# cvxopt/smcp

Hardware: AMD Instinct MI355X
Metric: Newton KKT solves/sec (higher is better)
Workload: dtype f64; 1 GPU; synth50k nested block-arrow SDP n=50000, 8073 cliques, m=100; kktsolver=chol, n=50000, cliques=8073, m=100, blkval_doubles=2493568, update_doubles=10689536, parallelism=single

## Files before the change

smcp_amd/csrc/capi.hip:

```cpp
#include <hip/hip_runtime.h>
#include <memory>
#include <unordered_map>

#include <algorithm>
#include <chrono>
#include <cstdio>
#include <cstring>
#include <map>
#include <new>
#include <atomic>
#include <thread>
#include <type_traits>
#include <vector>

#include "../../include/smcp_amd.h"
#include "context.hpp"
#include "switches.hpp"
#include "front_generic.hip"
#include "front_mfma.hip"
#include "front_large.hip"
#include "front_top.hip"
#include "front_inv.hip"
#include "front_n16.hip"
#include "front_downfam.hip"
// ... 336 lines not shown
  }
}

inline unsigned gather_parts(int namax, int64_t pairs = (int64_t)1 << 40, int ncu = 0) {
  const int base = std::max(1, std::min(64, (namax * namax) / (NT * 32)));
  if (pairs * base >= 2 * (int64_t)ncu) return (unsigned)base;
  const int cap = std::max(1, std::min(64, (namax * namax) / (NT * 2)));
  return (unsigned)std::max<int64_t>(base, std::min<int64_t>(cap, (2 * (int64_t)ncu + pairs - 1) / std::max<int64_t>(1, pairs)));
}
inline int namax_of(csp_ctx* c, const int32_t* lev) {
  const int64_t off = lev - c->D.levidx;
  const auto& lp = c->S.levptr;
  const int64_t l = std::upper_bound(lp.begin(), lp.end(), off) - lp.begin() - 1;
  return (l >= 0 && l < (int64_t)c->lev_namax.size()) ? c->lev_namax[l] : 0;
}

void gather_all(csp_ctx* c, const double* x, int64_t ldx, int nrhs, double* updbase, hipStream_t st) {
  TreeArgs a = tree_args(c);
  for_levels_down(c, [&](const int32_t* lev, int cnt) {
    a.lev = lev;
    launch(c, KID_gather_level, k_gather_level, dim3(cnt, nrhs, gather_parts(namax_of(c, lev), (int64_t)cnt * nrhs, c->D.ncu)), dim3(NT), st, a, x, ldx, updbase);
  });
}

int prepare_yaa(csp_ctx* c, const double* Y, bool need_fac, hipStream_t st, bool need_inv = false, bool allow_partial = false);
void complete_fac(csp_ctx* c, hipStream_t st);


constexpr size_t LDS_LIMIT = 160 * 1024 - 2048;

bool cache_off() {
  static int nocache = -1;
  if (nocache < 0) { const char* e = sw_str("SMCP_NOCACHE"); nocache = (e && e[0] == '1') ? 1 : 0; }
  return nocache == 1;
}

bool use_generic(const csp_ctx* c) {
  static int g = -1;
  if (g < 0) { const char* e = sw_str("SMCP_GENERIC"); g = (e && e[0] == '1') ? 1 : 0; }
  return g == 1 || (c && c->deterministic);
}

MfmaArgs mfma_args(csp_ctx* c, const double* ysc, int ymode, int nrhs) {
  MfmaArgs a;
  a.t = tree_args(c);
  a.t.lev = c->D.lev2idx;
  a.LK = c->D.lk;
  a.ysc = ysc;
  a.ymode = ymode;
  a.nnmax = a.namax = 0;
  a.nchmax = a.panmax = a.pkmax = a.plansum = 0;
  a.nrhs = nrhs;
  { static int sk = -1; if (sk < 0) { const char* e = sw_str("SMCP_SKIP"); sk = e ? atoi(e) : 0; } a.skip = sk; }
  a.dbg = (a.skip & 64) ? (unsigned long long*)(c->D.red + 768) : nullptr;
  a.lfd = c->D.lfd;
  a.dn = 0; a.dld = 0;
  a.kc_ptr = nullptr; a.kc_off = nullptr; a.kc_val = nullptr; a.kc_ids = nullptr;
  a.sp_rt = c->D.sp_rt; a.sp_mk = c->D.sp_mk;
  a.kc_stride = 0; a.kc_j0 = 0;
  a.nnmin = 0;
  a.grp_ptr = nullptr; a.grp_list = nullptr; a.chskip = nullptr; a.famt_ngrp = 0;
  a.fz_on = 0; a.fz_nat = 0; a.fz_cnn = 0; a.fz_stride = 0; a.fz_recl = 0;
  a.fz_tab = nullptr; a.fz_no = nullptr; a.fz_slot = nullptr; a.fz_ptr = nullptr; a.fz_pk = nullptr; a.fz_s = nullptr;
  a.level = 0; a.nS = 0; a.famna = a.fampan = a.fampk = a.famcna = a.famnn = a.famcnn = 0;
  return a;
}

int rhs_groups(int ncl, int nrhs, int target) {
  int g = (target + ncl - 1) / ncl;
  return std::max(1, std::min(g, nrhs));
}

template <class F>
void for_level_classes(csp_ctx* c, int64_t l, MfmaArgs a, F f, int set = 0) {
  const LevelClass& L = set ? c->sets[set].lvl[l] : c->lvl[l];
  const int32_t* base = set ? c->sets[set].lev2 + c->sets[set].off[l] : c->D.lev2idx + c->S.levptr[l];
  if (L.nI) {
    a.t.lev = base;
    a.nnmax = L.nnmaxI;
    a.namax = L.namaxI;
    a.nchmax = L.nchmaxI;
    a.panmax = L.panmaxI;
    a.pkmax = L.pkmaxI;
    a.plansum = L.plansumI;
    a.level = (int)l; a.nS = (int)L.nS; a.famna = L.famna; a.fampan = L.fampan; a.fampk = L.fampk; a.famcna = L.famcna; a.famnn = L.famnn; a.famcnn = L.famcnn;
    size_t lds = (size_t)mfma_lds_doubles(L.nnmaxI, L.namaxI) * sizeof(double);
    f(true, a, (int)L.nI, lds, lds > 48 * 1024 ? 512 : 256);
  }
  if (L.nII) {
    a.t.lev = base + L.nI;
    a.level = (int)l;
    a.nnmax = L.nnmaxII;
    a.nnmin = L.nnminII;
    a.namax = L.namaxII;
    a.nchmax = L.nchmaxII;
    f(false, a, (int)L.nII, (size_t)0, 1024);
  }
}


template <class F>
void for_all_large(csp_ctx* c, MfmaArgs a, F f) {
  if (!c->D.nII_total) return;
  a.t.lev = c->D.lev3idx + c->D.nI_total;
  a.nnmax = c->D.nnmaxII_all;
  a.namax = c->D.namaxII_all;
// ... 3332 lines not shown
```

smcp_amd/csrc/front_large.hip:

```cpp
#include <hip/hip_runtime.h>
#include <type_traits>

namespace smcp {

constexpr int LT = 64;
constexpr int LKC = 16;
constexpr int LSA = LT + 1, LSB = LKC + 1;

template <int PD>
__device__ inline double ldm(bool c, const double* p) {
  if constexpr (PD == 4) { const double v = *p; return c ? v : 0.0; }
  else return c ? *p : 0.0;
}
template <int PD = 1, class LA, class LB>
__device__ inline void gemm_tile64(d4 (&acc)[2][2], int M, int N, int Kd, int m0, int n0, LA la, LB lb,
                                   double* sA, double* sB, int kbeg = 0) {
  const int tid = threadIdx.x, lane = tid & 63, wave = tid >> 6;
  const int l15 = lane & 15, kq = lane >> 4;
  const int kfirst = (kbeg / LKC) * LKC;
  if (kfirst >= Kd) return;
  if constexpr (PD == 4) {
    const int wm = wave & 3, wn = wave >> 2;
    const int ia = tid & 63, ka = tid >> 6, kb = tid & 15, jb = tid >> 4;
    const int mi = max(0, min(m0 + ia, M - 1)), nj = max(0, min(n0 + jb, N - 1));
// ... 41 lines not shown
      vb[u] = (n0 + j < N && k0 + kb < Kd) ? lb(k0 + kb, n0 + j) : 0.0;
    }
  };
  fetch(kfirst);
  for (int k0 = kfirst; k0 < Kd; k0 += LKC) {
    __syncthreads();
#pragma unroll
    for (int u = 0; u < 4; ++u) {
      const int e = tid + 256 * u;
      sA[(e & 63) + (e >> 6) * LSA] = va[u];
      sB[(e & 15) + (e >> 4) * LSB] = vb[u];
    }
    __syncthreads();
    if (k0 + LKC < Kd) fetch(k0 + LKC);
#pragma unroll
    for (int ks = 0; ks < LKC / 4; ++ks) {
      const int kk = 4 * ks + kq;
      const double a0 = sA[(32 * wm + l15) + kk * LSA], a1 = sA[(32 * wm + 16 + l15) + kk * LSA];
      const double b0 = sB[kk + (32 * wn + l15) * LSB], b1 = sB[kk + (32 * wn + 16 + l15) * LSB];
      acc[0][0] = __builtin_amdgcn_mfma_f64_16x16x4f64(b0, a0, acc[0][0], 0, 0, 0);
      acc[1][0] = __builtin_amdgcn_mfma_f64_16x16x4f64(b0, a1, acc[1][0], 0, 0, 0);
      acc[0][1] = __builtin_amdgcn_mfma_f64_16x16x4f64(b1, a0, acc[0][1], 0, 0, 0);
      acc[1][1] = __builtin_amdgcn_mfma_f64_16x16x4f64(b1, a1, acc[1][1], 0, 0, 0);
    }
  }
  }
}
constexpr int LRC = 80;
constexpr int LCC = 18;
constexpr int LRC_DOUBLES = 4 * LKC * LRC;
__device__ inline bool rc_aligned(const double* p, int64_t ld) { return ((reinterpret_cast<uintptr_t>(p) & 15) == 0) && ((ld & 1) == 0); }
template <bool XC>
struct RcOperand {
  typedef double d2 __attribute__((ext_vector_type(2)));
  const double* p; int64_t step, second;
  int st0, st1;
  d2 r[2];
  __device__ inline void init(const double* X, int64_t ld) {
    const int tid = threadIdx.x;
    if constexpr (XC) {
      const int k2 = tid & 7, row = tid >> 3;
      p = X + 2 * k2 + (int64_t)row * ld; step = LKC; second = 32 * ld;
      st0 = 2 * k2 + row * LCC; st1 = st0 + 32 * LCC;
    } else {
      const int r2 = tid & 31, kk0 = tid >> 5;
      p = X + 2 * r2 + (int64_t)kk0 * ld; step = (int64_t)LKC * ld; second = 8 * ld;
      st0 = 2 * r2 + kk0 * LRC; st1 = st0 + 8 * LRC;
    }
  }
  __device__ inline void fetch() { r[0] = *reinterpret_cast<const d2*>(p); r[1] = *reinterpret_cast<const d2*>(p + second); p += step; }
  __device__ inline void stage(double* sX) const { *reinterpret_cast<d2*>(sX + st0) = r[0]; *reinterpret_cast<d2*>(sX + st1) = r[1]; }
  static __device__ inline double frag(const double* sX, int row, int kk) { return XC ? sX[kk + row * LCC] : sX[row + kk * LRC]; }
};
template <bool AC, bool BC>
__device__ inline void gemm_tile64_rc(d4 (&acc)[2][2], const double* A, int64_t lda, const double* B, int64_t ldb, int nk, double* smem) {
  constexpr int SL = LKC * LRC;
  const int tid = threadIdx.x, lane = tid & 63, wave = tid >> 6;
  const int l15 = lane & 15, kq = lane >> 4;
  const int wm = wave & 1, wn = wave >> 1;
  const int ns = nk / LKC;
  if (ns <= 0) return;
  RcOperand<AC> oa;
  RcOperand<BC> ob;
  oa.init(A, lda);
  ob.init(B, ldb);
  oa.fetch(); ob.fetch();
  __syncthreads();
  oa.stage(smem); ob.stage(smem + 2 * SL);
  __syncthreads();
  for (int s = 0; s < ns; ++s) {
    const double* sA = smem + (s & 1) * SL;
    const double* sB = smem + 2 * SL + (s & 1) * SL;
    if (s + 1 < ns) { oa.fetch(); ob.fetch(); }
#pragma unroll
    for (int ks = 0; ks < LKC / 4; ++ks) {
      const int kk = 4 * ks + kq;
      const double a0 = RcOperand<AC>::frag(sA, 32 * wm + l15, kk), a1 = RcOperand<AC>::frag(sA, 32 * wm + 16 + l15, kk);
      const double b0 = RcOperand<BC>::frag(sB, 32 * wn + l15, kk), b1 = RcOperand<BC>::frag(sB, 32 * wn + 16 + l15, kk);
      acc[0][0] = __builtin_amdgcn_mfma_f64_16x16x4f64(b0, a0, acc[0][0], 0, 0, 0);
      acc[1][0] = __builtin_amdgcn_mfma_f64_16x16x4f64(b0, a1, acc[1][0], 0, 0, 0);
      acc[0][1] = __builtin_amdgcn_mfma_f64_16x16x4f64(b1, a0, acc[0][1], 0, 0, 0);
      acc[1][1] = __builtin_amdgcn_mfma_f64_16x16x4f64(b1, a1, acc[1][1], 0, 0, 0);
    }
    if (s + 1 < ns) { oa.stage(smem + ((s + 1) & 1) * SL); ob.stage(smem + 2 * SL + ((s + 1) & 1) * SL); }
    __syncthreads();
  }
}
template <int PD, bool AC = false, bool BC = false>
__device__ inline void gemm_tile64_plain(d4 (&acc)[2][2], const double* A, int64_t lda, int M, const double* B, int64_t ldb, int N, int k0, int k1,
                                         int m0, int n0, double* smem) {
  if (k1 <= k0) return;
  if constexpr (PD == 1) {
    const double* A0 = AC ? A + k0 + (int64_t)m0 * lda : A + m0 + (int64_t)k0 * lda;
    const double* B0 = BC ? B + k0 + (int64_t)n0 * ldb : B + n0 + (int64_t)k0 * ldb;
    if (m0 + LT <= M && n0 + LT <= N && ((k1 - k0) % LKC) == 0 && (k0 % LKC) == 0 && rc_aligned(A0, lda) && rc_aligned(B0, ldb)) {
      gemm_tile64_rc<AC, BC>(acc, A0, lda, B0, ldb, k1 - k0, smem);
      return;
    }
  }
  gemm_tile64<PD>(acc, M, N, k1, m0, n0, [=](int m, int kk) { return AC ? A[kk + (int64_t)m * lda] : A[m + (int64_t)kk * lda]; },
                  [=](int kk, int n) { return BC ? B[kk + (int64_t)n * ldb] : B[n + (int64_t)kk * ldb]; }, smem, smem + LKC * LSA, k0);
}
__device__ inline bool tile64_pos(int a, int b, int r, int& m, int& n) {
  const int lane = threadIdx.x & 63, wave = threadIdx.x >> 6;
  const int l15 = lane & 15, kq = lane >> 4;
  if (blockDim.x == 1024) {
    m = 16 * (wave & 3) + l15; n = 16 * (wave >> 2) + kq + 4 * r;
    return a == 0 && b == 0;
  }
  m = 32 * (wave & 1) + 16 * a + l15; n = 32 * (wave >> 1) + 16 * b + kq + 4 * r;
  return true;
}
template <class F>
__device__ inline void tile64_foreach(const d4 (&acc)[2][2], int m0, int n0, int M, int N, F f) {
#pragma unroll
  for (int a = 0; a < 2; ++a)
#pragma unroll
    for (int b = 0; b < 2; ++b)
#pragma unroll
      for (int r = 0; r < 4; ++r) {
        int m, n;
        const bool has = tile64_pos(a, b, r, m, n);
        m += m0; n += n0;
        if (has && m < M && n < N) f(m, n, acc[a][b][r]);
      }
}
template <class LD, class ST>
__device__ inline void tile64_rmw(const d4 (&acc)[2][2], int m0, int n0, int M, int N, LD ld, ST st) {
  double old[2][2][4];
#pragma unroll
  for (int a = 0; a < 2; ++a)
#pragma unroll
    for (int b = 0; b < 2; ++b)
#pragma unroll
      for (int r = 0; r < 4; ++r) {
        int m, n;
        tile64_pos(a, b, r, m, n);
        old[a][b][r] = ld(max(0, min(m0 + m, M - 1)), max(0, min(n0 + n, N - 1)));
      }
#pragma unroll
  for (int a = 0; a < 2; ++a)
#pragma unroll
    for (int b = 0; b < 2; ++b)
#pragma unroll
      for (int r = 0; r < 4; ++r) {
        int m, n;
        const bool has = tile64_pos(a, b, r, m, n);
        m += m0; n += n0;
        if (has && m < M && n < N) st(m, n, acc[a][b][r], old[a][b][r]);
      }
}
__device__ inline void tile64_zero(d4 (&acc)[2][2]) {
#pragma unroll
  for (int a = 0; a < 2; ++a)
// ... 346 lines not shown
      const int cj = rel[j] - c0;
      const double* col = Uc + pk_col(j, nac) - j;
      for (int i = max(i0, j) + lane; i < i1; i += 64) unsafeAtomicAdd(&T[(rel[i] - r0) + cj * LF_TR], col[i]);
    }
  }
  __syncthreads();
  double* P = u + (int64_t)r * ldu + d.blk;
  double* U = a.t.upd + (int64_t)r * a.t.updlen + d.upd;
  const int nr = r1 - r0;
  for (int e = threadIdx.x; e < nr * (c1 - c0); e += blockDim.x) {
    const int i = r0 + e % nr, j = c0 + e / nr;
    if (i < j) continue;
    const double v = T[(i - r0) + (j - c0) * LF_TR];
    if (j < nn) {
      if (v != 0.0) P[i + (int64_t)j * nf] += (sgn == 1) ? -v : v;
    } else if (sgn) {
      if (v != 0.0) U[(i - nn) + (int64_t)(j - nn) * na] += v;
    } else {
      U[(i - nn) + (int64_t)(j - nn) * na] = v;
    }
  }
}
__global__ void k_lf_zero_skipped(MfmaArgs a) {
  const CliqueDesc d = a.t.cl[a.t.lev[blockIdx.x]];
  const int r = blockIdx.y;
  for (int q = d.chbeg; q < d.chend; ++q) {
    const int ck = a.t.chidx[q];
    if (!a.chskip[ck]) continue;
    const CliqueDesc c = a.t.cl[ck];
    double* UP = a.t.updp + (int64_t)r * a.t.updplen + c.updp;
    for (int e = threadIdx.x; e < c.na * (c.na + 1) / 2; e += blockDim.x) UP[e] = 0.0;
  }
}
__global__ void k_lf_clear_upd(MfmaArgs a) {
  const int k = a.t.lev[blockIdx.y];
  const CliqueDesc d = a.t.cl[k];
  double* U = a.t.upd + (int64_t)blockIdx.z * a.t.updlen + d.upd;
  const int64_t len = (int64_t)d.na * d.na;
  for (int64_t e = (int64_t)blockIdx.x * blockDim.x + threadIdx.x; e < len; e += (int64_t)gridDim.x * blockDim.x) U[e] = 0.0;
}

__host__ __device__ inline bool lf_sym_split(int nn) { return nn > 6 * LT; }
template <int PD>
__global__ void __launch_bounds__(PD == 4 ? 1024 : 256, 4) k_lf_up1(MfmaArgs a, double* u, int64_t ldu) {
  __shared__ __attribute__((aligned(16))) double smem[PD == 1 ? LRC_DOUBLES : LKC * LSA + LT * LSB];
  double* const sA = smem; double* const sB = smem + LKC * LSA;
  const LfCtx c = lf_ctx(a, u, ldu);
  const int nn = c.nn, na = c.na, nf = c.nf;
  const int mtA = tiles64(na), ntN = tiles64(nn);
  const int nE = mtA * ntN, nT = ntN * ntN;
  const int t = blockIdx.x;
  if (t >= nE + nT) return;
  const double* P = c.P;
  auto fsym = [=](int kk, int n) { return P[max(kk, n) + (int64_t)min(kk, n) * nf]; };
  d4 acc[2][2];
  tile64_zero(acc);
  if (t < nE) {
    const int m0 = (t % mtA) * LT, n0 = (t / mtA) * LT;
    const double* K = c.K;
    gemm_tile64<PD>(acc, na, nn, nn, m0, n0, [=](int m, int kk) { return K[m + (int64_t)kk * nf]; }, fsym, sA, sB);
    double* E = c.E; double* Pw = c.P;
    tile64_rmw(acc, m0, n0, na, nn, [=](int m, int n) { return Pw[nn + m + (int64_t)n * nf]; },
               [=](int m, int n, double v, double f) {
                 E[m + (int64_t)n * na] = f - 0.5 * v;
                 Pw[nn + m + (int64_t)n * nf] = f - v;
               });
  } else {
    const int tt = t - nE, m0 = (tt % ntN) * LT, n0 = (tt / ntN) * LT;
    const double* Li = c.Li;
    if (n0 > m0) return;
    if (lf_sym_split(nn)) {
      gemm_tile64<PD>(acc, nn, nn, min(nn, n0 + LT), m0, n0, [=](int m, int kk) { return Li[m + (int64_t)kk * nf]; },
                  [=](int kk, int n) { const double v_ = ldm<PD>(kk >= n, &P[kk + (int64_t)n * nf]); return kk == n ? 0.5 * v_ : v_; },
                  sA, sB, n0);
      gemm_tile64_plain<PD, false, true>(acc, Li, nf, nn, P, nf, nn, n0 + LT, min(nn, m0 + LT), m0, n0, smem);
    } else {
      gemm_tile64<PD>(acc, nn, nn, min(nn, m0 + LT), m0, n0, [=](int m, int kk) { return Li[m + (int64_t)kk * nf]; }, fsym, sA, sB);
    }
    double* T = c.T;
    tile64_foreach(acc, m0, n0, nn, nn, [=](int m, int n, double v) { T[m + (int64_t)n * nn] = v; });
  }
}
constexpr int LF_ZSP_MAXNN = 7168;
__global__ void __launch_bounds__(256) k_lf_zsp(MfmaArgs a, double* u, int64_t ldu) {
  extern __shared__ __attribute__((aligned(16))) double zc[];
  __shared__ int s_row[64];
  __shared__ double s_w[64];
  const LfCtx c = lf_ctx(a, u, ldu);
  const int nn = c.nn, nf = c.nf;
  const int col = blockIdx.x;
  if (col >= nn) return;
  const int tid = threadIdx.x;
  const int r0 = (col / LT) * LT;
  const int r = blockIdx.z;
  const int j = a.kc_ids ? a.kc_ids[a.kc_j0 + r] : a.kc_j0 + r;
  const int32_t* kp = a.kc_ptr + (int64_t)c.k * a.kc_stride;
  const int e0 = kp[j], e1 = kp[j + 1];
  auto lower = [&](int64_t key) {
    int lo = e0, hi = e1;
    while (lo < hi) { const int mid = (lo + hi) >> 1; if ((int64_t)a.kc_off[mid] < key) lo = mid + 1; else hi = mid; }
    return lo;
  };
  const int b0 = lower((int64_t)col * nf), b1 = lower((int64_t)(col + 1) * nf);
  for (int i = r0 + tid; i < nn; i += 256) zc[i] = 0.0;
  const double* Li = c.Li;
  for (int base = b0; base < b1; base += 64) {
    __syncthreads();
    if (tid < 64 && base + tid < b1) {
      const int off = a.kc_off[base + tid];
      const int row = off - col * nf;
      s_row[tid] = row;
      s_w[tid] = row == col ? 0.5 * a.kc_val[base + tid] : a.kc_val[base + tid];
    }
    __syncthreads();
    const int ne = min(64, b1 - base);
    for (int q = 0; q < ne; ++q) {
      const int row = s_row[q];
      const double w = s_w[q];
      const double* Lc = Li + (int64_t)row * nf;
      int i = r0 + tid;
      if (i < row) i += ((row - i + 255) >> 8) << 8;
      for (; i + 768 < nn; i += 1024) {
        const double v0 = Lc[i], v1 = Lc[i + 256], v2 = Lc[i + 512], v3 = Lc[i + 768];
        zc[i] += w * v0; zc[i + 256] += w * v1; zc[i + 512] += w * v2; zc[i + 768] += w * v3;
      }
      for (; i < nn; i += 256) zc[i] += w * Lc[i];
    }
  }
  double* T = c.T + (int64_t)col * nn;
  for (int i = r0 + tid; i < nn; i += 256) T[i] = zc[i];
}
template <int PD>
__global__ void __launch_bounds__(PD == 4 ? 1024 : 256, 4) k_lf_up2(MfmaArgs a, double* u, int64_t ldu) {
  __shared__ __attribute__((aligned(16))) double smem[PD == 1 ? LRC_DOUBLES : LKC * LSA + LT * LSB];
  const LfCtx c = lf_ctx(a, u, ldu);
  const int nn = c.nn, na = c.na, nf = c.nf;
  const int mtA = tiles64(na), ntN = tiles64(nn);
  const int nU = mtA * (mtA + 1) / 2, nG = mtA * ntN, nN = ntN * (ntN + 1) / 2;
  const int t = blockIdx.x;
  if (t >= nU + nG + nN) return;
  const double* K = c.K; const double* E = c.E; const double* Li = c.Li; const double* T = c.T; const double* P = c.P;
  d4 acc[2][2];
  tile64_zero(acc);
  if (t < nU) {
    int tm, tn;
    lower_pair(t, tm, tn);
    const int m0 = tm * LT, n0 = tn * LT;
    gemm_tile64_plain<PD>(acc, K, nf, na, E, na, na, 0, nn, m0, n0, smem);
    gemm_tile64_plain<PD>(acc, E, na, na, K, nf, na, 0, nn, m0, n0, smem);
    const double* U = c.U; double* UP = c.UP;
    if (c.hasch)
      tile64_rmw(acc, m0, n0, na, na, [=](int m, int n) { return U[m + (int64_t)n * na]; },
                 [=](int m, int n, double v, double uo) { if (m >= n) UP[pk_idx(m, n, na)] = uo - v; });
    else
      tile64_foreach(acc, m0, n0, na, na, [=](int m, int n, double v) {
        if (m >= n) UP[pk_idx(m, n, na)] = -v;
      });
  } else if (t < nU + nG) {
    const int tt = nG - 1 - (t - nU), m0 = (tt % mtA) * LT, n0 = (tt / mtA) * LT;
    gemm_tile64_plain<PD>(acc, P + nn, nf, na, Li, nf, nn, 0, min(nn, n0 + LT), m0, n0, smem);
    double* G = c.G;
    tile64_foreach(acc, m0, n0, na, nn, [=](int m, int n, double v) { G[m + (int64_t)n * na] = v; });
  } else {
    int tm, tn;
    lower_pair_wide_first(t - nU - nG, ntN, tm, tn);
    const int m0 = tm * LT, n0 = tn * LT;
    gemm_tile64_plain<PD>(acc, T, nn, nn, Li, nf, nn, 0, min(nn, n0 + LT), m0, n0, smem);
    if (lf_sym_split(nn))
      gemm_tile64_plain<PD>(acc, Li, nf, nn, T, nn, nn, 0, min(nn, n0 + LT), m0, n0, smem);
    double* Pw = c.P;
    tile64_foreach(acc, m0, n0, nn, nn, [=](int m, int n, double v) { if (m >= n) Pw[m + (int64_t)n * nf] = v; });
  }
}
template <int PD>
__global__ void __launch_bounds__(PD == 4 ? 1024 : 256, 4) k_lf_up3(MfmaArgs a, double* u, int64_t ldu) {
  __shared__ double sA[LKC * LSA], sB[LT * LSB];
#ifdef SMCP_STAMPS
  const bool stamp = a.dbg && threadIdx.x == 0 && blockIdx.x == 0 && blockIdx.y == 0 && blockIdx.z == 0 && a.nrhs == 1;
  unsigned long long ts0 = stamp ? wall_clock64() : 0, ts1 = 0, ts2 = 0;
#endif
  const LfCtx c = lf_ctx(a, u, ldu);
  const int nn = c.nn, na = c.na, nf = c.nf;
  const int mtA = tiles64(na), ntN = tiles64(nn);
  const int t = blockIdx.x;
  if (t >= mtA * ntN) return;
  const int m0 = (t % mtA) * LT, n0 = (t / mtA) * LT;
  const double* G = c.G; const double* Y = c.Ys;
  double* Pw = c.P;
  const int ymode = a.ymode;
  d4 acc[2][2];
  tile64_zero(acc);
  if (ymode) {
#ifdef SMCP_STAMPS
    if (stamp) ts1 = wall_clock64();
#endif
    gemm_tile64<PD>(acc, na, nn, (ymode == 1 || ymode == 2) ? na : min(na, m0 + LT), m0, n0,
                [=](int m, int kk) { return yacc<PD>(Y, na, ymode, m, kk); },
                [=](int kk, int n) { return G[kk + (int64_t)n * na]; }, sA, sB, ymode == 2 ? m0 : 0);
#ifdef SMCP_STAMPS
    if (stamp) ts2 = wall_clock64();
#endif
    tile64_foreach(acc, m0, n0, na, nn, [=](int m, int n, double v) { Pw[nn + m + (int64_t)n * nf] = v; });
#ifdef SMCP_STAMPS
    if (stamp) {
      __builtin_amdgcn_s_waitcnt(0);
      const unsigned long long ts3 = wall_clock64();
      atomicAdd(a.dbg + 26, ts1 - ts0); atomicAdd(a.dbg + 27, ts2 - ts1); atomicAdd(a.dbg + 28, ts3 - ts2); atomicAdd(a.dbg + 29, 1ull);
    }
#endif
  } else {
    tile64_rmw(acc, m0, n0, na, nn, [=](int m, int n) { return G[m + (int64_t)n * na]; },
               [=](int m, int n, double, double g) { Pw[nn + m + (int64_t)n * nf] = g; });
  }
}

template <int PD>
__global__ void __launch_bounds__(PD == 4 ? 1024 : 256, 4) k_lf_down1(MfmaArgs a, double* u, int64_t ldu) {
  __shared__ __attribute__((aligned(16))) double smem[PD == 1 ? LRC_DOUBLES : LKC * LSA + LT * LSB];
  double* const sA = smem; double* const sB = smem + LKC * LSA;
  const LfCtx c = lf_ctx(a, u, ldu);
  const int nn = c.nn, na = c.na, nf = c.nf;
  const int mtA = tiles64(na), ntN = tiles64(nn);
  const int nE = mtA * ntN, nT = ntN * ntN;
  const int t = blockIdx.x;
  if (t >= nE + nT) return;
  const double* P = c.P; const double* Li = c.Li;
  auto li = [=](int kk, int n) { return Li[kk + (int64_t)n * nf]; };
  d4 acc[2][2];
  tile64_zero(acc);
  if (t < nE) {
    const int m0 = (t % mtA) * LT, n0 = (t / mtA) * LT;
    gemm_tile64_plain<PD, false, true>(acc, P + nn, nf, na, Li, nf, nn, n0, nn, m0, n0, smem);
    double* E = c.E;
    tile64_foreach(acc, m0, n0, na, nn, [=](int m, int n, double v) { E[m + (int64_t)n * na] = v; });
  } else {
    const int tt = t - nE, m0 = (tt % ntN) * LT, n0 = (tt / ntN) * LT;
    if (lf_sym_split(nn)) {
      if (n0 > m0) return;
      gemm_tile64_plain<PD, false, true>(acc, P, nf, nn, Li, nf, nn, n0, m0, m0, n0, smem);
      gemm_tile64<PD>(acc, nn, nn, min(nn, m0 + LT), m0, n0,
                  [=](int m, int kk) { const double v_ = ldm<PD>(m >= kk, &P[m + (int64_t)kk * nf]); return m == kk ? 0.5 * v_ : v_; }, li, sA, sB, m0);
    } else {
      gemm_tile64<PD>(acc, nn, nn, nn, m0, n0,
                  [=](int m, int kk) { return P[max(m, kk) + (int64_t)min(m, kk) * nf]; }, li, sA, sB, n0);
    }
    double* T = c.T;
    tile64_foreach(acc, m0, n0, nn, nn, [=](int m, int n, double v) { T[m + (int64_t)n * nn] = v; });
  }
// ... 1103 lines not shown
```

smcp_amd/csrc/front_mfma.hip:

```cpp
#include <hip/hip_runtime.h>

namespace smcp {

typedef double d4 __attribute__((ext_vector_type(4)));

template <class FA, class FB, class FC>
__device__ inline void wg_mma(int M, int N, int Kd, FA A, FB B, FC store, bool lower_only = false, int rot = 0) {
  const int lane = threadIdx.x & 63, nw = blockDim.x >> 6;
  const int wave = ((threadIdx.x >> 6) + nw - (rot % nw)) % nw;
  const int mt = (M + 15) >> 4, nt = (N + 15) >> 4;
  const int l15 = lane & 15, kq = lane >> 4;
  for (int t = wave; t < mt * nt; t += nw) {
    const int tm = t % mt, tn = t / mt;
    if (lower_only && tm < tn) continue;
    const int m = tm * 16 + l15, nb = tn * 16 + l15;
    d4 acc = {0.0, 0.0, 0.0, 0.0};
    constexpr int KU = 2;
    for (int k0 = 0; k0 < Kd; k0 += 4 * KU) {
      double av[KU], bv[KU];
#pragma unroll
      for (int u = 0; u < KU; ++u) {
        const int k = k0 + 4 * u + kq;
        const bool kin = k < Kd;
        av[u] = (kin && m < M) ? A(m, k) : 0.0;
        bv[u] = (kin && nb < N) ? B(k, nb) : 0.0;
      }
#pragma unroll
      for (int u = 0; u < KU; ++u)
        if (k0 + 4 * u < Kd) acc = __builtin_amdgcn_mfma_f64_16x16x4f64(bv[u], av[u], acc, 0, 0, 0);
    }
#pragma unroll
    for (int r = 0; r < 4; ++r) {
      const int n = tn * 16 + kq + 4 * r;
      if (m < M && n < N) store(m, n, acc[r]);
    }
  }
}

template <int UNR, class LoadF, class UseF>
__device__ inline void batched_loop(int begin, int end, int step, LoadF load, UseF use) {
  for (int e0 = begin; e0 < end; e0 += step * UNR) {
    decltype(load(0)) v[UNR];
#pragma unroll
    for (int u = 0; u < UNR; ++u) {
      const int e = e0 + u * step;
      if (e < end) v[u] = load(e);
    }
#pragma unroll
    for (int u = 0; u < UNR; ++u) {
      const int e = e0 + u * step;
      if (e < end) use(e, v[u]);
    }
  }
}

struct MfmaArgs {
  TreeArgs t;
  const double* LK;
  const double* ysc;
  int ymode;
  int nnmax, namax;
  int nrhs;
  int nchmax, panmax, pkmax, plansum;
  int skip;
  unsigned long long* dbg;
  double* lfd;
  int dn; int64_t dld;
  const int32_t* kc_ptr; const int32_t* kc_off; const double* kc_val; const int32_t* kc_ids;
  int kc_stride, kc_j0;
  const double* sp_rt; const double* sp_mk;
  int level, nS, famna, fampan, fampk, famcna, famnn, famcnn;
  int nnmin;
  const int32_t* grp_ptr; const int32_t* grp_list; const uint8_t* chskip;
  int famt_ngrp;
  int fz_on, fz_nat, fz_cnn, fz_stride;
  int64_t fz_recl;
  const double* fz_tab; const int32_t* fz_no; const int32_t* fz_slot; const int32_t* fz_ptr; const int32_t* fz_pk; const double* fz_s;
};

__device__ __host__ inline int padld(int x) { return x | 1; }

__host__ __device__ inline int64_t mfma_lds_doubles(int nn, int na) {
  int64_t lk = padld(na), ll = padld(nn), lf = padld(nn + na);
  int64_t nnc = nn;
  return lk * nnc + ll * nnc + lk * (int64_t)na + lf * nnc + ll * nnc + lk * nnc + lk * nnc + ll * nnc + lk * (int64_t)na + 16 * 16 + 8 + (na + 2) / 2;
}

enum : int { WK_K = 1, WK_LI = 2, WK_Y = 4, WK_F = 8, WK_FNN = 16, WK_E = 32, WK_G = 64, WK_T = 128, WK_U = 256, WK_ALL = 511 };
constexpr int WK_CHOL = WK_F | WK_U;
constexpr int WK_PINV = WK_K | WK_LI | WK_E | WK_U;
constexpr int WK_DOWN0 = WK_ALL & ~(WK_Y | WK_FNN);
constexpr int WK_COMPL = WK_Y | WK_F | WK_FNN | WK_E | WK_G | WK_T;
__host__ __device__ inline int64_t mfma_lds_doubles_for(int mask, int nn, int na) {
  const int64_t lk = padld(na), ll = padld(nn), lf = padld(nn + na), nnc = nn;
  int64_t t = 0;
  if (mask & WK_K) t += lk * nnc;
  if (mask & WK_LI) t += ll * nnc;
  if (mask & WK_Y) t += lk * (int64_t)na;
  if (mask & WK_F) t += lf * nnc;
  if (mask & WK_FNN) t += ll * nnc;
  if (mask & WK_E) t += lk * nnc;
  if (mask & WK_G) t += lk * nnc;
  if (mask & WK_T) t += ll * nnc;
  if (mask & WK_U) t += lk * (int64_t)na;
  return t + 16 * 16 + 8 + (na + 2) / 2;
}
__host__ __device__ inline int64_t completion_lds_doubles(int nn, int na) {
  return mfma_lds_doubles_for(WK_COMPL, nn, na) + (nn > 16 ? 16 * 128 : 0);
}

struct Work {
  const double* K; int ldk;
  const double* Li; int ldl;
  const double* Y; int ldy;
  double* F; int ldf;
  double* Fnn; int ldn;
  double* E; int lde;
// ... 1272 lines not shown
```

smcp_amd/csrc/switches.hpp:

```cpp
#pragma once
#include <cstdio>
#include <cstdlib>
#include <cstring>
#include <string>

extern char** environ;

namespace smcp {

struct Switch { const char* name; const char* dflt; const char* doc; };

static const Switch SWITCHES[] = {
  {"SMCP_GENERIC", "0", "1: any-size fixed-order kernels of front_generic.hip for every tree operation (as CSP_TUNE_DETERMINISTIC)"},
  {"SMCP_LARGE", "1", "0: no tiled large-front kernels (fronts beyond LDS take the one-workgroup HBM kernels)"},
  {"SMCP_NOCACHE", "0", "1: nothing derived from (L, Y) is reused between calls"},
  {"SMCP_FORK", "1", "0: no side streams, everything on the caller's stream"},
  {"SMCP_AUX_PRIO", "1", "0: side stream 0 (few-workgroup chains) at default instead of highest priority"},
  {"SMCP_AUX_PRIO1", "1", "0: side stream 1 (filler work) at default instead of lowest priority"},
  {"SMCP_EVENT_SYSFENCE", "0", "1: internal events with the default system-scope release (12 us per hand-over instead of 7)"},
  {"SMCP_SCALING_OVERLAP", "1", "0: csp_cholesky_projected_inverse as its three steps one after the other"},
  {"SMCP_CHOL_PREP", "1", "0: k_prep_lk in a launch of its own instead of inside k_chol_mfma (narrow supernodes)"},
  {"SMCP_FAC_PARTIAL", "1", "0: chol(Y_AA) of the family children always formed by the fused scaling point"},
  {"SMCP_MID", "1", "0: per-step kernels instead of k_mid_chol / k_lf_diag_inv for fronts of at most 272 rows"},
  {"SMCP_TOP_FUSED", "1", "0: k_mid_chol, and k_lf_diag_inv / k_lf_trtri for the inverse at the scaling point, instead of the register-resident k_top_chol for fronts of at most 208 rows"},
  {"SMCP_TRTRI", "1", "0: block-row triangular inversion of large fronts instead of recursive doubling"},
  {"SMCP_N16", "1", "0: no shape-specialised k_hess_up_n16"},
  {"SMCP_OLDLDS", "0", "1: k_hess_up_mfma<true> instead of the padded / n16 kernels"},
  {"SMCP_DOWN_W", "1", "0: k_hess_down_mfma instead of the one-wave k_hess_down_w"},
  {"SMCP_DOWN_FAM", "1", "most right-hand sides of a root -> leaves sweep that take the one-launch family kernel k_hess_down_fam (0: never; the per-level k_hess_down_w launches)"},
  {"SMCP_UP_FAM", "1", "most dense right-hand sides of a leaves -> root sweep that take the resident family kernel k_hess_up_fam1, the level-0 cliques outside the families riding along (0: never; k_hess_up_fam and a launch of their own for those cliques)"},
  {"SMCP_FAM", "1", "0: no family kernels (per-level sweeps with the update exchange through HBM)"},
  {"SMCP_FAM2", "1", "0: no sparse-input family kernels (k_fam_sparse, k_fam_terms): k_hess_up_fam"},
  {"SMCP_FAMT", "1", "0: no entry-driven family sweep k_fam_terms (k_fam_sparse instead)"},
  {"SMCP_FZ", "1", "0: the family parents' packed updates go through HBM (k_fam_terms writes, the extend-add reads) instead of being formed by k_lf_assemble_fz"},
  {"SMCP_FAMT_GROUP", "1", "0: no sibling groups of family parents (k_fam_terms_grp)"},
  {"SMCP_LFSP", "1", "0: dense phases instead of the sparse-input sweep k_lfsp_up of childless large fronts"},
  {"SMCP_LFSP_GROUP", "1", "0: no sibling groups in k_lfsp_up"},
  {"SMCP_ZSP", "1", "0: dense first phase of wide childless fronts instead of k_lf_zsp"},
  {"SMCP_LEAFGRAM", "1", "0: never the closed-form Gram blocks of the family children (k_leaf_tables / k_leaf_pairs)"},
  {"SMCP_LG_SIDE", "1", "0: leaf Gram blocks after the sweep on the caller's stream instead of beside the top phases"},
  {"SMCP_GRAM_EARLY", "0", "1: the Gram chunks of the levels 0 / 1 rows on the side branch beside the top fronts' phase kernels (measured slower: 3.37 against 3.22 ms per step)"},
  {"SMCP_LG_EARLY", "1", "0: leaf Gram blocks beside the phase kernels of the top fronts instead of from the start of the sweep"},
  {"SMCP_FACI_LDS", "1", "0: inverse Y_AA factors of the small fronts by block rows against HBM (k_factor_inverse) instead of in LDS"},
  {"SMCP_FZ_TAIL", "1", "0: every (front, right-hand side) pair of the fused extend-add is one workgroup's task, also in a thin last round"},
  {"SMCP_GRAM", "1", "0: reference (two-sweep) formulation of the Schur complement instead of the Gram formulation"},
  {"SMCP_SCM", "1", "0: column-sparse constraints swept like the others (no SCMcolumn2 route)"},
  {"SMCP_TRSM_MM", "1", "0: csp_trsm through the generic level kernels instead of tile products"},
  {"SMCP_TRMM_MM", "1", "0: no MFMA tile products in csp_trmm (every front on the FMA kernels); 2: tile products for the large fronts only, also from 32 columns on"},
  {"SMCP_SYR2K_MM", "1", "0: no MFMA tile products in csp_syr2k (every front on the FMA kernel); 2: tile products for the large fronts only, whatever the rank (read on every call)"},
  {"SMCP_SYMM_MM", "1", "0: no MFMA tile products in csp_symm (every front on the FMA kernel); 2: tile products for the large fronts only, whatever the column count (read on every call)"},
  {"SMCP_POTRS_MANY_MM", "1", "0: no MFMA tile products in the block steps of dense_potrs_many / kkt_solve_many (FMA updates whatever the column count; read on every call)"},
  {"SMCP_ALDS", "1", "0: extend-add of large fronts by gather plan only (no LDS streaming kernel)"},
  {"SMCP_ALDS_DYN", "1", "0: one workgroup per (front, right-hand side) instead of the task-drawing grid"},
  {"SMCP_ALDS_FILL", "1", "0: k_panel_fill builds the input panels instead of the extend-add (sgn 3)"},
  {"SMCP_ASM", "plan", "t: tiled extend-add kernel instead of the gather plan"},
  {"SMCP_ROOT_FUSED", "0", "1: fused two-product sweep of fronts without separator (Y_NN explicit: condition squared; studies only)"},
  {"SMCP_PD", "0", "1: four-wave tile products everywhere (no sixteen-wave shape for small launches)"},
  {"SMCP_POTRF_OLD", "0", "1: generic one-workgroup dense Cholesky"},
  {"SMCP_FLOW", "1", "0: no one-launch blocked Cholesky with in-launch tile dataflow (front_flow.hip): per-step kernels for dense matrices / single fronts beyond 272 rows"},
  {"SMCP_FLOW_WG", "112", "workgroups of that launch (at most 112: four launches fit the chip side by side)"},
  {"SMCP_POTRS_OLD", "0", "1: generic one-workgroup dense solve"},
  {"SMCP_POTRS_STEPS", "0", "1: per-block launches of the dense solve instead of k_dense_potrs_one"},
  {"SMCP_POTRF_DEFER", "1", "0: kkt_schur_factor factors H at once even under deferred status"},
  {"SMCP_QR_TRSM", "mfma", "f: vector-FMA substitution kernel of kkt_qr instead of the MFMA one"},
  {"SMCP_FTHR_CHOL", "128", "threads of k_chol_mfma on the leaf class"},
  {"SMCP_FTHR_PINV", "256", "threads of k_pinv_mfma on the leaf class"},
  {"SMCP_FTHR_YAA", "64", "threads of k_factor_yaa_lds on the leaf class"},
  {"SMCP_FTHR_YAA_MID", "256", "threads of k_factor_yaa_lds on separator blocks of 33 .. 64 rows"},
  {"SMCP_N16_THR_LEAF", "128", "threads of k_hess_up_n16 for one or two right-hand sides on childless fronts"},
  {"SMCP_DIAG_THREADS", "512", "threads of k_lf_diag"},
  {"SMCP_POTRF_THREADS", "1024", "threads of k_dense_potrf_small"},
  {"SMCP_FZ_THREADS", "1024", "threads of k_lf_assemble_fz (512: eight waves, no register spills, slower)"},
  {"SMCP_PD_WGS", "1", "largest launch, in workgroups per CU, that takes the sixteen-wave tile shape"},
  {"SMCP_ALDS_Z", "0", "workgroups per (front, right-hand side) of the LDS extend-add (0: automatic)"},
  {"SMCP_RHS_SPLIT", "16", "fewest right-hand sides for the two-stream split of a large-front sweep (plain extend-add launch only)"},
  {"SMCP_RHS_PARTS", "2", "parts of that split (2 or 3)"},
  {"SMCP_RHS_SPLIT_DYN", "0", "1: the split also with the task-drawing extend-add"},
// ... 53 lines not shown
```

Measured before the change: 345.3 KKT solves/s.

## Use 16-byte-load tile products for symmetric and triangular operands in large-front kernels

Adds RcSymOperand and RcTriOperand loaders so the symmetric F_NN product in k_lf_up1 and the triangular R^T product in k_lf_up3 can use the vectorized double-buffered gemm_tile64_ops path instead of the per-element lambda loader. Edge tiles are shifted inward (ms/ns clamped) so full 64x64 tiles apply, and writes are masked back to the original region. The intent is to cut scalar global loads and address arithmetic in the top-front GEMMs. The cost is more code paths, redundant compute on overlapping edge tiles, and a default-on switch to fall back.

```diff
diff --git a/smcp_amd/csrc/capi.hip b/smcp_amd/csrc/capi.hip
--- a/smcp_amd/csrc/capi.hip
+++ b/smcp_amd/csrc/capi.hip
@@ -412,6 +412,7 @@
   a.nchmax = a.panmax = a.pkmax = a.plansum = 0;
   a.nrhs = nrhs;
   { static int sk = -1; if (sk < 0) { const char* e = sw_str("SMCP_SKIP"); sk = e ? atoi(e) : 0; } a.skip = sk; }
+  { static int tp = -1; if (tp < 0) tp = sw_on("SMCP_TOP_PLAIN", 1); a.top_plain = tp; }
   a.dbg = (a.skip & 64) ? (unsigned long long*)(c->D.red + 768) : nullptr;
   a.lfd = c->D.lfd;
   a.dn = 0; a.dld = 0;
diff --git a/smcp_amd/csrc/front_large.hip b/smcp_amd/csrc/front_large.hip
--- a/smcp_amd/csrc/front_large.hip
+++ b/smcp_amd/csrc/front_large.hip
@@ -117,18 +117,61 @@
   __device__ inline void stage(double* sX) const { *reinterpret_cast<d2*>(sX + st0) = r[0]; *reinterpret_cast<d2*>(sX + st1) = r[1]; }
   static __device__ inline double frag(const double* sX, int row, int kk) { return XC ? sX[kk + row * LCC] : sX[row + kk * LRC]; }
 };
-template <bool AC, bool BC>
-__device__ inline void gemm_tile64_rc(d4 (&acc)[2][2], const double* A, int64_t lda, const double* B, int64_t ldb, int nk, double* smem) {
+struct RcTriOperand {
+  RcOperand<true> o;
+  int kd0;
+  __device__ inline void init(const double* X, int64_t ld) { o.init(X, ld); kd0 = 2 * (threadIdx.x & 7) - (threadIdx.x >> 3); }
+  __device__ inline void fetch() {
+    o.fetch();
+    o.r[0].x = kd0 >= 0 ? o.r[0].x : 0.0; o.r[0].y = kd0 + 1 >= 0 ? o.r[0].y : 0.0;
+    o.r[1].x = kd0 >= 32 ? o.r[1].x : 0.0; o.r[1].y = kd0 + 1 >= 32 ? o.r[1].y : 0.0;
+    kd0 += LKC;
+  }
+  __device__ inline void stage(double* sX) const { o.stage(sX); }
+  static __device__ inline double frag(const double* sX, int row, int kk) { return RcOperand<true>::frag(sX, row, kk); }
+};
+struct RcSymOperand {
+  typedef double d2 __attribute__((ext_vector_type(2)));
+  const double* D; int64_t ld;
+  const double* pr; const double* pc;
+  int kb;
+  int rn, rst;
+  int cn, cst;
+  d2 rr[2], rc[2]; double rt;
+  __device__ inline void init(const double* X, int64_t ld_) {
+    const int tid = threadIdx.x;
+    D = X; ld = ld_; kb = 0;
+    const int r2 = tid & 31, kk0 = tid >> 5;
+    rn = 2 * r2; pr = X + rn + (int64_t)kk0 * ld; rst = rn + kk0 * LRC;
+    const int k2 = tid & 7, row = tid >> 3;
+    cn = row; pc = X + 2 * k2 + (int64_t)row * ld; cst = row + 2 * k2 * LRC;
+  }
+  __device__ inline void fetch() {
+    const int tk = threadIdx.x & 15, tj = threadIdx.x >> 4;
+    if (rn >= kb + LKC) { rr[0] = *reinterpret_cast<const d2*>(pr); rr[1] = *reinterpret_cast<const d2*>(pr + 8 * ld); }
+    if (cn < kb) rc[0] = *reinterpret_cast<const d2*>(pc);
+    if (cn + 32 < kb) rc[1] = *reinterpret_cast<const d2*>(pc + 32 * ld);
+    rt = D[kb + max(tk, tj) + (int64_t)(kb + min(tk, tj)) * ld];
+    pr += (int64_t)LKC * ld; pc += LKC; kb += LKC;
+  }
+  __device__ inline void stage(double* sX) const {
+    const int tk = threadIdx.x & 15, tj = threadIdx.x >> 4;
+    const int k0 = kb - LKC;
+    if (rn >= k0 + LKC) { *reinterpret_cast<d2*>(sX + rst) = rr[0]; *reinterpret_cast<d2*>(sX + rst + 8 * LRC) = rr[1]; }
+    if (cn < k0) { sX[cst] = rc[0].x; sX[cst + LRC] = rc[0].y; }
+    if (cn + 32 < k0) { sX[cst + 32] = rc[1].x; sX[cst + 32 + LRC] = rc[1].y; }
+    sX[k0 + tj + tk * LRC] = rt;
+  }
+  static __device__ inline double frag(const double* sX, int row, int kk) { return RcOperand<false>::frag(sX, row, kk); }
+};
+template <class OA, class OB>
+__device__ inline void gemm_tile64_ops(d4 (&acc)[2][2], OA& oa, OB& ob, int nk, double* smem) {
   constexpr int SL = LKC * LRC;
   const int tid = threadIdx.x, lane = tid & 63, wave = tid >> 6;
   const int l15 = lane & 15, kq = lane >> 4;
   const int wm = wave & 1, wn = wave >> 1;
   const int ns = nk / LKC;
   if (ns <= 0) return;
-  RcOperand<AC> oa;
-  RcOperand<BC> ob;
-  oa.init(A, lda);
-  ob.init(B, ldb);
   oa.fetch(); ob.fetch();
   __syncthreads();
   oa.stage(smem); ob.stage(smem + 2 * SL);
@@ -140,8 +183,8 @@
 #pragma unroll
     for (int ks = 0; ks < LKC / 4; ++ks) {
       const int kk = 4 * ks + kq;
-      const double a0 = RcOperand<AC>::frag(sA, 32 * wm + l15, kk), a1 = RcOperand<AC>::frag(sA, 32 * wm + 16 + l15, kk);
-      const double b0 = RcOperand<BC>::frag(sB, 32 * wn + l15, kk), b1 = RcOperand<BC>::frag(sB, 32 * wn + 16 + l15, kk);
+      const double a0 = OA::frag(sA, 32 * wm + l15, kk), a1 = OA::frag(sA, 32 * wm + 16 + l15, kk);
+      const double b0 = OB::frag(sB, 32 * wn + l15, kk), b1 = OB::frag(sB, 32 * wn + 16 + l15, kk);
       acc[0][0] = __builtin_amdgcn_mfma_f64_16x16x4f64(b0, a0, acc[0][0], 0, 0, 0);
       acc[1][0] = __builtin_amdgcn_mfma_f64_16x16x4f64(b0, a1, acc[1][0], 0, 0, 0);
       acc[0][1] = __builtin_amdgcn_mfma_f64_16x16x4f64(b1, a0, acc[0][1], 0, 0, 0);
@@ -150,6 +193,14 @@
     if (s + 1 < ns) { oa.stage(smem + ((s + 1) & 1) * SL); ob.stage(smem + 2 * SL + ((s + 1) & 1) * SL); }
     __syncthreads();
   }
+}
+template <bool AC, bool BC>
+__device__ inline void gemm_tile64_rc(d4 (&acc)[2][2], const double* A, int64_t lda, const double* B, int64_t ldb, int nk, double* smem) {
+  RcOperand<AC> oa;
+  RcOperand<BC> ob;
+  oa.init(A, lda);
+  ob.init(B, ldb);
+  gemm_tile64_ops(acc, oa, ob, nk, smem);
 }
 template <int PD, bool AC = false, bool BC = false>
 __device__ inline void gemm_tile64_plain(d4 (&acc)[2][2], const double* A, int64_t lda, int M, const double* B, int64_t ldb, int N, int k0, int k1,
@@ -165,6 +216,24 @@
   }
   gemm_tile64<PD>(acc, M, N, k1, m0, n0, [=](int m, int kk) { return AC ? A[kk + (int64_t)m * lda] : A[m + (int64_t)kk * lda]; },
                   [=](int kk, int n) { return BC ? B[kk + (int64_t)n * ldb] : B[n + (int64_t)kk * ldb]; }, smem, smem + LKC * LSA, k0);
+}
+template <int PD>
+__device__ inline void gemm_tile64_symb(d4 (&acc)[2][2], const double* A, int64_t lda, int M, const double* P, int nf, int nn, int k1,
+                                        int m0, int n0, double* smem, bool plain) {
+  if constexpr (PD == 1) {
+    if (plain && m0 + LT <= M && n0 + LT <= nn && k1 >= n0 + LT && (k1 % LKC) == 0 && (n0 % LKC) == 0 && rc_aligned(A + m0, lda) && rc_aligned(P, nf)) {
+      gemm_tile64_rc<false, false>(acc, A + m0, lda, P + n0, nf, n0, smem);
+      RcOperand<false> oa;
+      RcSymOperand ob;
+      oa.init(A + m0 + (int64_t)n0 * lda, lda);
+      ob.init(P + n0 + (int64_t)n0 * nf, nf);
+      gemm_tile64_ops(acc, oa, ob, LT, smem);
+      gemm_tile64_rc<false, true>(acc, A + m0 + (int64_t)(n0 + LT) * lda, lda, P + n0 + LT + (int64_t)n0 * nf, nf, k1 - n0 - LT, smem);
+      return;
+    }
+  }
+  gemm_tile64<PD>(acc, M, nn, k1, m0, n0, [=](int m, int kk) { return A[m + (int64_t)kk * lda]; },
+                  [=](int kk, int n) { return P[max(kk, n) + (int64_t)min(kk, n) * nf]; }, smem, smem + LKC * LSA);
 }
 __device__ inline bool tile64_pos(int a, int b, int r, int& m, int& n) {
   const int lane = threadIdx.x & 63, wave = threadIdx.x >> 6;
@@ -617,33 +686,37 @@
   const int t = blockIdx.x;
   if (t >= nE + nT) return;
   const double* P = c.P;
-  auto fsym = [=](int kk, int n) { return P[max(kk, n) + (int64_t)min(kk, n) * nf]; };
-  d4 acc[2][2];
-  tile64_zero(acc);
-  if (t < nE) {
-    const int m0 = (t % mtA) * LT, n0 = (t / mtA) * LT;
-    const double* K = c.K;
-    gemm_tile64<PD>(acc, na, nn, nn, m0, n0, [=](int m, int kk) { return K[m + (int64_t)kk * nf]; }, fsym, sA, sB);
+  d4 acc[2][2];
+  tile64_zero(acc);
+  const bool isE = t < nE;
+  const int tt = isE ? t : t - nE, mt = isE ? mtA : ntN;
+  const int m0 = (tt % mt) * LT, n0 = (tt / mt) * LT;
+  if (!isE && n0 > m0) return;
+  int ms = m0, ns = n0;
+  if constexpr (PD == 1) {
+    const int Mr = isE ? na : nn;
+    if (a.top_plain && !lf_sym_split(nn) && Mr >= LT && nn >= LT) { ms = min(m0, Mr - LT); ns = min(n0, nn - LT); }
+  }
+  if (!isE && lf_sym_split(nn)) {
+    const double* Li = c.Li;
+    gemm_tile64<PD>(acc, nn, nn, min(nn, n0 + LT), m0, n0, [=](int m, int kk) { return Li[m + (int64_t)kk * nf]; },
+                [=](int kk, int n) { const double v_ = ldm<PD>(kk >= n, &P[kk + (int64_t)n * nf]); return kk == n ? 0.5 * v_ : v_; },
+                sA, sB, n0);
+    gemm_tile64_plain<PD, false, true>(acc, Li, nf, nn, P, nf, nn, n0 + LT, min(nn, m0 + LT), m0, n0, smem);
+  } else {
+    gemm_tile64_symb<PD>(acc, isE ? c.K : c.Li, nf, isE ? na : nn, P, nf, nn, isE ? nn : min(nn, ms + LT), ms, ns, smem, a.top_plain != 0);
+  }
+  if (isE) {
     double* E = c.E; double* Pw = c.P;
-    tile64_rmw(acc, m0, n0, na, nn, [=](int m, int n) { return Pw[nn + m + (int64_t)n * nf]; },
+    tile64_rmw(acc, ms, ns, na, nn, [=](int m, int n) { return Pw[nn + m + (int64_t)n * nf]; },
                [=](int m, int n, double v, double f) {
+                 if (m < m0 || n < n0) return;
                  E[m + (int64_t)n * na] = f - 0.5 * v;
                  Pw[nn + m + (int64_t)n * nf] = f - v;
                });
   } else {
-    const int tt = t - nE, m0 = (tt % ntN) * LT, n0 = (tt / ntN) * LT;
-    const double* Li = c.Li;
-    if (n0 > m0) return;
-    if (lf_sym_split(nn)) {
-      gemm_tile64<PD>(acc, nn, nn, min(nn, n0 + LT), m0, n0, [=](int m, int kk) { return Li[m + (int64_t)kk * nf]; },
-                  [=](int kk, int n) { const double v_ = ldm<PD>(kk >= n, &P[kk + (int64_t)n * nf]); return kk == n ? 0.5 * v_ : v_; },
-                  sA, sB, n0);
-      gemm_tile64_plain<PD, false, true>(acc, Li, nf, nn, P, nf, nn, n0 + LT, min(nn, m0 + LT), m0, n0, smem);
-    } else {
-      gemm_tile64<PD>(acc, nn, nn, min(nn, m0 + LT), m0, n0, [=](int m, int kk) { return Li[m + (int64_t)kk * nf]; }, fsym, sA, sB);
-    }
     double* T = c.T;
-    tile64_foreach(acc, m0, n0, nn, nn, [=](int m, int n, double v) { T[m + (int64_t)n * nn] = v; });
+    tile64_foreach(acc, ms, ns, nn, nn, [=](int m, int n, double v) { if (m >= m0 && n >= n0) T[m + (int64_t)n * nn] = v; });
   }
 }
 constexpr int LF_ZSP_MAXNN = 7168;
@@ -739,7 +812,8 @@
 }
 template <int PD>
 __global__ void __launch_bounds__(PD == 4 ? 1024 : 256, 4) k_lf_up3(MfmaArgs a, double* u, int64_t ldu) {
-  __shared__ double sA[LKC * LSA], sB[LT * LSB];
+  __shared__ __attribute__((aligned(16))) double smem[PD == 1 ? LRC_DOUBLES : LKC * LSA + LT * LSB];
+  double* const sA = smem; double* const sB = smem + LKC * LSA;
 #ifdef SMCP_STAMPS
   const bool stamp = a.dbg && threadIdx.x == 0 && blockIdx.x == 0 && blockIdx.y == 0 && blockIdx.z == 0 && a.nrhs == 1;
   unsigned long long ts0 = stamp ? wall_clock64() : 0, ts1 = 0, ts2 = 0;
@@ -759,6 +833,20 @@
 #ifdef SMCP_STAMPS
     if (stamp) ts1 = wall_clock64();
 #endif
+    bool fast = false;
+    if constexpr (PD == 1) {
+      fast = a.top_plain && ymode == 2 && m0 + LT <= na && n0 + LT <= nn && (na % LKC) == 0 &&
+             rc_aligned(Y + m0 + (int64_t)m0 * na, na) && rc_aligned(G + m0 + (int64_t)n0 * na, na);
+      if (fast) {
+        RcTriOperand oa;
+        RcOperand<true> ob;
+        oa.init(Y + m0 + (int64_t)m0 * na, na);
+        ob.init(G + m0 + (int64_t)n0 * na, na);
+        gemm_tile64_ops(acc, oa, ob, LT, smem);
+        gemm_tile64_rc<true, true>(acc, Y + m0 + LT + (int64_t)m0 * na, na, G + m0 + LT + (int64_t)n0 * na, na, na - m0 - LT, smem);
+      }
+    }
+    if (!fast)
     gemm_tile64<PD>(acc, na, nn, (ymode == 1 || ymode == 2) ? na : min(na, m0 + LT), m0, n0,
                 [=](int m, int kk) { return yacc<PD>(Y, na, ymode, m, kk); },
                 [=](int kk, int n) { return G[kk + (int64_t)n * na]; }, sA, sB, ymode == 2 ? m0 : 0);
diff --git a/smcp_amd/csrc/front_mfma.hip b/smcp_amd/csrc/front_mfma.hip
--- a/smcp_amd/csrc/front_mfma.hip
+++ b/smcp_amd/csrc/front_mfma.hip
@@ -63,6 +63,7 @@
   int nrhs;
   int nchmax, panmax, pkmax, plansum;
   int skip;
+  int top_plain;
   unsigned long long* dbg;
   double* lfd;
   int dn; int64_t dld;
diff --git a/smcp_amd/csrc/switches.hpp b/smcp_amd/csrc/switches.hpp
--- a/smcp_amd/csrc/switches.hpp
+++ b/smcp_amd/csrc/switches.hpp
@@ -23,6 +23,7 @@
   {"SMCP_FAC_PARTIAL", "1", "0: chol(Y_AA) of the family children always formed by the fused scaling point"},
   {"SMCP_MID", "1", "0: per-step kernels instead of k_mid_chol / k_lf_diag_inv for fronts of at most 272 rows"},
   {"SMCP_TOP_FUSED", "1", "0: k_mid_chol, and k_lf_diag_inv / k_lf_trtri for the inverse at the scaling point, instead of the register-resident k_top_chol for fronts of at most 208 rows"},
+  {"SMCP_TOP_PLAIN", "1", "0: the element-loader tile product for F_NN in k_lf_up1 and R^T in k_lf_up3 of multi-right-hand-side sweeps instead of the 16-byte-load product with RcSymOperand / RcTriOperand"},
   {"SMCP_TRTRI", "1", "0: block-row triangular inversion of large fronts instead of recursive doubling"},
   {"SMCP_N16", "1", "0: no shape-specialised k_hess_up_n16"},
   {"SMCP_OLDLDS", "0", "1: k_hess_up_mfma<true> instead of the padded / n16 kernels"},
```

New measurement: 348.4 KKT solves/s (median of 3 runs). No clear change (+0.9%).
